# stevengiacalone/triceratops

Hardware: AMD Instinct MI355X
Metric: light-curve-point x sample evals/sec (higher is better)
Workload: dtype f64

## Files before the change

### include/trx_debug.h

```cpp
#ifndef TRX_DEBUG_H
#define TRX_DEBUG_H

#include "trx.h"

#ifdef __cplusplus
extern "C" {
#endif

int trx_set_rows_per_wave(int rows);
int trx_set_cell_packing_below(int n_time);
int trx_debug_batch_plan(long rows, int rows_per_wave, int taper, long* positions, int* rows_min);

int trx_set_supersample_tiers(int on);
int trx_set_stencil(int on);
int trx_set_skip_excluded(int on);
int trx_set_debug_node_counts(int on);
int trx_set_kepler_stepping(int on);

int trx_set_bounded_evaluation(int mode);
int trx_set_debug_bounded_lnl(int on);
int trx_set_debug_poison(int on);
int trx_set_debug_bug(int on);
int trx_set_probe_rows(int rows);
int trx_set_star_chain(int on);
int trx_set_row_order(int on);
int trx_debug_row_order(long* n_rows, long* segment_capacity, int* counts, int* lists, double* row_blocks);
int trx_set_whole_trips(int on);
int trx_set_one_sweep(int mode);
int trx_set_full_chunks(int mode);
long trx_debug_cells_lds_one_row(void);
int trx_debug_whole_trips(long* whole, long* walked, int reset);
int trx_debug_chain_counts(long* chains, long* calls_in_chains, long* posterior_calls_in_chains, int reset);

int trx_debug_select_from_halfchi2(const double* halfchi2, const double* lnprior, const double* cols,
                                   const double* cols_pad, long n, long N, long n_total, int ncol, int twin, int K,
                                   int moments, double lnsigma, double* out_record, double* out_post_x,
                                   double* out_table, void* stream);

int trx_debug_capture_buffers(long* live, long* idle);

#ifdef __cplusplus
}
#endif
#endif
```

### triceratops_amd/_lib.py

```python
import ctypes
import os
import threading

import numpy as np
import torch

_HERE = os.path.dirname(os.path.abspath(__file__))
LIB_PATH = os.environ.get("TRX_LIB") or os.path.join(_HERE, "libtrx.so")
TESTING_LIB_PATH = os.environ.get("TRX_TESTING_LIB") or os.path.join(_HERE, "libtrx_testing.so")

MODEL_TP, MODEL_EB, MODEL_EB_TWIN, MODEL_RAW = 0, 1, 2, 3
FLAG_COMPANION_IS_HOST, FLAG_SCALAR_K, FLAG_FP32_MODEL, FLAG_EVALUATE_EXCLUDED = 1, 2, 4, 8
FLAG_ALL_SUBEXPOSURES, FLAG_NO_STENCIL, FLAG_COUNT_EVALUATIONS, FLAG_FULL_EVALUATION = 16, 32, 64, 128
FLAG_WEIGHT_MOMENTS = 256
N_PARAM = {MODEL_TP: 10, MODEL_EB: 11, MODEL_EB_TWIN: 11, MODEL_RAW: 9}
ERR_NTOTAL = 4

ABI_SYMBOLS = (
    "trx_lnl_batch", "trx_lnl_batch_weighted", "trx_flux_grid", "trx_chi2_grid", "trx_chi2_grid_weighted",
    "trx_chi2_grid_offset", "trx_chi2_grid_baseline", "trx_workspace_bytes",
    "trx_log_mean_exp", "trx_lnz_scenario", "trx_lnz_from_halfchi2", "trx_lnz_moments_from_halfchi2",
    "trx_posterior_from_halfchi2", "trx_grid_quantiles",
    "trx_lnl_batch_host", "trx_flux_grid_host",
    "trx_log_mean_exp_host", "trx_skipped_rows", "trx_pruned_rows",
    "trx_draw_scenario", "trx_draw_args_size", "trx_scenario_evidence", "trx_scenario_enqueue", "trx_star_enqueue",
    "trx_scenario_args_size", "trx_release_scratch", "trx_version", "trx_last_error", "trx_device_count",
)
WARP_SYMBOLS = ("trxw_hist_from_halfchi2",)
NOISE_SYMBOLS = ("trxn_chi2_grid_ou",)
MIX_SYMBOLS = ("trxm_chi2_grid_ou_mix",)
SHIFT_SYMBOLS = ("trxt_softmin_rows",)
ROBUST_SYMBOLS = ("trxr_chi2_grid_robust",)
GLS_SYMBOLS = ("trxg_chi2_grid_ou_baseline",)
SS_SYMBOLS = ("trxs_chi2_grid_ss2",)
WHITE_SYMBOLS = ("trxv_chi2_grid_white_mix",)
DEBUG_SYMBOLS = (
    "trx_set_rows_per_wave", "trx_set_cell_packing_below", "trx_debug_batch_plan", "trx_set_supersample_tiers",
    "trx_set_stencil", "trx_set_skip_excluded", "trx_set_debug_node_counts", "trx_set_kepler_stepping",
    "trx_set_bounded_evaluation", "trx_set_debug_bounded_lnl", "trx_set_debug_poison", "trx_set_debug_bug",
    "trx_set_probe_rows", "trx_set_star_chain", "trx_debug_capture_buffers", "trx_debug_chain_counts",
    "trx_set_row_order", "trx_debug_row_order", "trx_set_whole_trips", "trx_debug_whole_trips", "trx_set_one_sweep",
    "trx_set_full_chunks", "trx_debug_cells_lds_one_row", "trx_debug_select_from_halfchi2",
)


class TrxError(RuntimeError):
    pass


EXTRA_FLAGS = 0
CELL_PACKING_BELOW = 320
STATS = {"rows": 0, "cells": 0, "launches": 0, "native_calls": 0}
_stats_lock = threading.Lock()


def count_launch(rows, n_time):
    with _stats_lock:
        STATS["rows"] += rows
        STATS["cells"] += rows * n_time
        STATS["launches"] += 1
TRACE = None
TRACE_SAMPLE_ROWS = 128


def reset_stats():
# ... 109 lines not shown
    L.trxs_chi2_grid_ss2.argtypes = [_vp, _vp, c_int, c_long, _vp, c_double, c_int, _vp, _vp, _vp, _vp, _vp]
    L.trx_grid_quantiles.restype = c_int
    L.trx_grid_quantiles.argtypes = [_vp, c_long, c_int, _vp, _vp, c_long, _vp, c_int, _vp, _vp]
    L.trx_lnl_batch_host.restype = c_int
    L.trx_lnl_batch_host.argtypes = [c_int, c_int, _vp, _vp, c_int, c_double, _vp, c_long,
                                     c_double, c_int, _vp]
    L.trx_flux_grid_host.restype = c_int
    L.trx_flux_grid_host.argtypes = [c_int, c_int, _vp, c_int, _vp, c_long, c_double, c_int, _vp, _vp]
    L.trx_log_mean_exp_host.restype = c_int
    L.trx_log_mean_exp_host.argtypes = [_vp, c_long, c_long, _vp]
    L.trx_skipped_rows.restype = c_int
    L.trx_skipped_rows.argtypes = [ctypes.POINTER(ctypes.c_ulonglong), c_int]
    L.trx_pruned_rows.restype = c_int
    L.trx_pruned_rows.argtypes = [ctypes.POINTER(ctypes.c_ulonglong), c_int]
    L.trx_version.restype = ctypes.c_char_p
    L.trx_last_error.restype = ctypes.c_char_p
    L.trx_device_count.restype = c_int
    L.trx_testing = bool(testing)
    if testing:
        for name in ("trx_set_rows_per_wave", "trx_set_kepler_stepping", "trx_set_skip_excluded",
                     "trx_set_bounded_evaluation", "trx_set_debug_bounded_lnl", "trx_set_debug_poison",
                     "trx_set_debug_bug", "trx_set_star_chain", "trx_set_probe_rows", "trx_set_stencil",
                     "trx_set_supersample_tiers", "trx_set_debug_node_counts", "trx_set_cell_packing_below",
                     "trx_set_row_order", "trx_set_whole_trips", "trx_set_one_sweep", "trx_set_full_chunks"):
            fn = getattr(L, name)
            fn.restype = c_int
            fn.argtypes = [c_int]
        L.trx_debug_cells_lds_one_row.restype = c_long
        L.trx_debug_cells_lds_one_row.argtypes = []
        L.trx_debug_capture_buffers.restype = c_int
        L.trx_debug_capture_buffers.argtypes = [ctypes.POINTER(c_long), ctypes.POINTER(c_long)]
        L.trx_debug_row_order.restype = c_int
        L.trx_debug_row_order.argtypes = [ctypes.POINTER(c_long), ctypes.POINTER(c_long), _vp, _vp, _vp]
        L.trx_debug_whole_trips.restype = c_int
        L.trx_debug_whole_trips.argtypes = [ctypes.POINTER(c_long), ctypes.POINTER(c_long), c_int]
        L.trx_debug_select_from_halfchi2.restype = c_int
        L.trx_debug_select_from_halfchi2.argtypes = [_vp, _vp, _vp, _vp, c_long, c_long, c_long, c_int, c_int, c_int, c_int,
                                                     c_double, _vp, _vp, _vp, _vp]
    return L


def check(rc):
    if rc:
        msg = lib().trx_last_error().decode()
        if rc == ERR_NTOTAL:
            raise ValueError(msg)
        raise TrxError("libtrx error %d: %s" % (rc, msg))


def version():
    return lib().trx_version().decode()


_gpu_seen = False


def require_gpu():
    global _gpu_seen
# ... 141 lines not shown

def debug_row_order():
    L = lib()
    assert L.trx_testing, "debug_row_order needs use_testing_library()"
    n, cap = ctypes.c_long(0), ctypes.c_long(0)
    check(L.trx_debug_row_order(ctypes.byref(n), ctypes.byref(cap), None, None, None))
    counts = np.zeros(64, dtype=np.int32)
    lists = np.zeros(64 * cap.value, dtype=np.int32)
    blocks = np.zeros((n.value, 19), dtype=np.float64)
    check(L.trx_debug_row_order(ctypes.byref(n), ctypes.byref(cap), counts.ctypes.data, lists.ctypes.data,
                                blocks.ctypes.data))
    lists = lists.reshape(64, cap.value)
    return counts.reshape(16, 4), [lists[s, :max(0, min(int(counts[s]), cap.value))].copy() for s in range(64)], blocks


def debug_whole_trips(reset=False):
    L = lib()
    assert L.trx_testing, "debug_whole_trips needs use_testing_library()"
    whole, walked = ctypes.c_long(0), ctypes.c_long(0)
    check(L.trx_debug_whole_trips(ctypes.byref(whole), ctypes.byref(walked), 1 if reset else 0))
    return whole.value, walked.value


def lnl_batch_weighted(model, flags, time_d, flux_d, inv_var_d, params_d, exptime, nsamples, sec_limit=float("inf"),
                       out=None):
    require_gpu()
    n, nt = params_d.shape[1], time_d.numel()
    assert params_d.shape[0] == N_PARAM[model] and params_d.is_contiguous()
    assert flux_d.numel() == nt and inv_var_d.numel() == nt
    assert time_d.is_contiguous() and flux_d.is_contiguous() and inv_var_d.is_contiguous()
    accumulate = out is not None
    if out is None:
        out = torch.empty(n, dtype=torch.float64, device=params_d.device)
    assert out.shape == (n,) and out.dtype == torch.float64 and out.is_contiguous()
    if n == 0:
        return out
    with torch.cuda.device(params_d.device):
        check(lib().trx_lnl_batch_weighted(model, flags, time_d.data_ptr(), flux_d.data_ptr(), inv_var_d.data_ptr(),
                                           nt, params_d.data_ptr(), n, float(exptime), int(nsamples),
                                           float(sec_limit), int(accumulate), out.data_ptr(), _stream(params_d)))
    return out


def flux_grid(model, flags, time_d, params_d, exptime, nsamples, want_secdepth=True, out=None):
    require_gpu()
    n = params_d.shape[1]
# ... 312 lines not shown
```

### triceratops_amd/csrc/trx_cells.hpp

```cpp
#pragma once
#include <hip/hip_runtime.h>
#include <math.h>

#include <cstddef>
#include <cstdint>

#include "../../include/trx.h"
#include "trx_device.hpp"
#include "trx_internal.hpp"

namespace {

using namespace trx;

constexpr int MODE_LNL = 0;
constexpr int MODE_GRID = 1;

struct RowsArgs {
    int model, flags;
    const double* time;
    const double* flux;
    int n_time;
    double sigma;
    const double* params;
// ... 105 lines not shown
__device__ unsigned long long g_phase_cycles[8];
#define TRX_TICK(var) const unsigned long long var = __builtin_readcyclecounter()
#define TRX_TOCK(slot, from) tm[slot] += __builtin_readcyclecounter() - (from)
#else
#define TRX_TICK(var)
#define TRX_TOCK(slot, from)
#endif

#ifdef TRX_TAIL_TIMERS
constexpr int kTailWaves = 1 << 17;
__device__ unsigned long long g_tail[4] = {~0ull, 0ull, 0ull, 0ull};
__device__ unsigned long long g_tail_finish[kTailWaves];
#endif

constexpr int kStatShards = 256, kStatPad = 16;
__device__ unsigned long long g_row_stats[2][kStatShards][kStatPad];
__device__ __forceinline__ void add_row_stat(int which, unsigned count)
{
    if (count) atomicAdd(&g_row_stats[which][(blockIdx.x + 41u * blockIdx.y) & (kStatShards - 1)][0], (unsigned long long)count);
}

#ifdef TRX_TESTING
__device__ unsigned long long g_trip_stats[2][kStatShards][kStatPad];
__device__ __forceinline__ void add_trip_stat(int which, unsigned count)
{
    if (count) atomicAdd(&g_trip_stats[which][(blockIdx.x + 41u * blockIdx.y) & (kStatShards - 1)][0], (unsigned long long)count);
}
__device__ __forceinline__ bool whole_trips_on(const RowsArgs& a) { return a.whole_trips != 0; }
__device__ __forceinline__ bool one_sweep_on(const RowsArgs& a, bool lnl) { return a.one_sweep >= (lnl ? 1 : 2); }
__device__ __forceinline__ bool full_chunks_on(const RowsArgs& a, bool lnl) { return a.full_chunks >= (lnl ? 1 : 2); }
#define TRX_TRIP_STAT(var) ++var
#else
__device__ __forceinline__ bool whole_trips_on(const RowsArgs&) { return true; }
__device__ __forceinline__ bool one_sweep_on(const RowsArgs&, bool lnl) { return lnl; }
__device__ __forceinline__ bool full_chunks_on(const RowsArgs&, bool lnl) { return lnl; }
#define TRX_TRIP_STAT(var)
#endif

__device__ __forceinline__ double k_rule(double k, bool scalar_rule)
{
    if (scalar_rule) { if (fabs(k - 1.0) < 1e-6) k *= 0.999; }
    else             { if ((k - 1.0) < 1e-6) k *= 0.999; }
    return k;
}

#ifndef TRX_BATCH_WAVES
#define TRX_BATCH_WAVES 4
#endif

constexpr int kBatchWaves = TRX_BATCH_WAVES;
__host__ __device__ constexpr int cells_waves(bool long_rows) { return long_rows ? 1 : kBatchWaves; }
#ifndef TRX_TIER_LDS
#define TRX_TIER_LDS(PRUNE, LONG) true
#endif
#ifndef TRX_ATAN_TAB
#define TRX_ATAN_TAB(PRUNE, LONG) (((PRUNE) && !(LONG)) ? 2 : 1)
#endif
#ifndef TRX_LONG_ROWS_IN_LDS
// ... 519 lines not shown
}

struct BranchMap {
    unsigned char id[TRX_CHAIN_MAX_BRANCHES];
};
__global__ __launch_bounds__(64) void sec_scan_kernel_star(RowsArgs common, BranchTab bt, BranchMap map)
{
    const RowsArgs a = star_args(common, bt, 0, (int)map.id[blockIdx.y]);
    if (!a.need_sec) return;
    sec_scan_body<8>(a);
}
static_assert(offsetof(RowC, excl) == (kRowDoubles - 1) * sizeof(double), "excl is the last field of RowC");

struct CellState {
    double sE[64], cE[64];
    double t[64];
    double facc[64];
    unsigned meta[64];
    union {
        unsigned short rel[64];
        double held[2 * kStM];
    };
};
struct StencilState {
    double fc[64 + 2 * kStM];
    double stw[2 * kStM + 1];
};
constexpr int kFcB = 2 * kStM;
constexpr int kCentreNode = 1023;

__device__ __forceinline__ double fp32_model_slack(double lb, int n_probed, double rs2)
{
    return 1e-5 * sqrt(2.0 * (double)n_probed * rs2 * fmax(lb, 0.0));
}

template <int BITS>
__device__ __forceinline__ int lane_prefix(int cnt, int& total)
{
    int off = 0;
    total = 0;
#pragma unroll
    for (int b = 0; b < BITS; ++b) {
        const unsigned long long m = __ballot((cnt >> b) & 1);
        off += lanes_below(m) << b;
        total += __popcll(m) << b;
    }
// ... 113 lines not shown
{
    typedef const __attribute__((address_space(4))) T* KernArgs;
    KernArgs p = (KernArgs)__builtin_amdgcn_kernarg_segment_ptr();
    asm volatile("" : "+s"(p));
    return (const T*)p;
}

template <int MODE, bool STEP, bool FP32, bool LONG, bool ST, bool PRUNE, int ARGS = 0, bool WT = false>
__device__ __forceinline__ void cells_body(const RowsArgs& a_in, const double st_radius)
{
    constexpr int kReload = TRX_ARGS_RELOAD ? ARGS : 0;
    const RowsArgs& a = a_in;
    static_assert(!PRUNE || (MODE == MODE_LNL && !ST), "bounded evaluation: likelihood mode, no stencil");
    static_assert(!WT || (MODE == MODE_LNL && !PRUNE), "per-point weights: likelihood mode, full evaluation");
    extern __shared__ double lds_all[];
#ifdef TRX_TAIL_TIMERS
    const unsigned long long tail_start = LONG ? wall_clock64() : 0ull;
#endif
    constexpr bool kOrdered = LONG && !PRUNE && !WT && MODE == MODE_LNL;
    int ordered_row = -2;
    if (kOrdered && a.order) ordered_row = (int)row_order_at(a.order, (long)blockIdx.x, a.n, (int)threadIdx.x);
    constexpr bool kCarry = TRX_CARRY_CELLS && STEP && !LONG;
    constexpr bool kLazyTiers = TRX_LAZY_TIERS && ST && STEP && LONG && !PRUNE;
    constexpr int W = cells_waves(LONG);
    const int wave = W > 1 ? __builtin_amdgcn_readfirstlane((int)(threadIdx.x >> 6)) : 0;
    double* tier_xw = lds_all;
    double* atab = tier_xw + 2 * kTiers * kTierMaxNodes;
    double* thead = atab + kAtanRanges * kAtanCols;
    double* lds = lds_all + a.wave_off + (size_t)wave * a.wave_doubles;
    const int Bl = LONG ? 1 : a.B;
    RowC* rows = reinterpret_cast<RowC*>(lds);
    double* hacc = lds + (size_t)Bl * kRowDoubles;
    double* hmout = hacc + Bl;
    double* hrem = hmout + Bl;
    double* hlp = hrem + Bl;
    unsigned short* pdesc = reinterpret_cast<unsigned short*>(hlp + Bl);
    constexpr int kCellsWindow = cells_window(LONG);
    unsigned short* winlist = pdesc + kCellsPairs;
    CellState& cs = *reinterpret_cast<CellState*>(winlist + kCellsWindow);
    StencilState& ss = *reinterpret_cast<StencilState*>(&cs + 1);
    const double* tl = LONG ? a.time : (lds_all + a.tl_off);
    const double* fl = LONG ? a.flux : (tl + a.n_time);
    const double* wl = LONG ? a.inv_var : (fl + a.n_time);
    if (a.use_tiers) {
        for (int i = threadIdx.x; i < 2 * kTiers * kTierMaxNodes; i += 64 * W) tier_xw[i] = a.tier_xw[i];
    }
// ... 51 lines not shown
        const unsigned long long* const surv_count = a.surv_count;
        if (a.part == 1) row1 = np;
        else if (a.part == 2) {
            if (a.split && hdr[kHdrProbe] != 0.0) { rlist = probe_list; row1 = (long)*probe_count; }
            else row0 = np;
        }
        else if (hdr[kHdrProbe] != 0.0) { rlist = surv_list; row1 = (long)*surv_count; }
        else row0 = np;
        if (!LONG && (a.part == 3 || (a.part == 2 && rlist))) B = listed_pass_rows(a, row1 - row0, a.part);
        if (!LONG && a.part == 1 && a.split) B = kPilotB < Bl ? kPilotB : Bl;
        nbatch = (row1 - row0 + B - 1) / B;
    }
    const bool third_two = PRUNE && !LONG && a.part == 3 && a.pstride3 > 1;
    const int pstride = third_two ? a.pstride3 : a.pstride;
    const bool probing = PRUNE && pstride > 1 && hdr[kHdrProbe] != 0.0 &&
                         (a.part == 0 || a.part == 2 || third_two);
    if (PRUNE && a.split && a.part == 2 && !probing) return;
    const BatchPlan bp = LONG ? BatchPlan{} : batch_plan(uniform_long(row1 - row0), __builtin_amdgcn_readfirstlane(B), !PRUNE);
    const long positions = LONG ? (nbatch + 7) / 8 : bp.P;
    const long v0 = (long)(blockIdx.x & 7) + 8 * ((long)(blockIdx.x >> 3) * W + wave);
    unsigned n_skipped = 0, n_pruned = 0;
#ifdef TRX_TESTING
    unsigned n_whole = 0, n_walked = 0;
#endif
    for (long v = v0; v < 8 * positions; v += (long)gridDim.x * W) {
        RowsArgs a_again;
        if (kReload == 2) {
            const StarKernArgs* k = kernel_arguments<StarKernArgs>();
            a_again = star_args(k->common, k->bt, k->part);
        }
        const RowsArgs& a = (kReload == 1) ? *kernel_arguments<RowsArgs>() : ((kReload == 2) ? a_again : a_in);
        long base;
        int nb;
        if (kOrdered && ordered_row != -2) {
            if (v != v0 || ordered_row < 0) continue;
            base = (long)ordered_row;
            nb = 1;
        } else if (LONG) {
            const long batch = (v & 7) * positions + (v >> 3);
            if ((v >> 3) >= positions || batch >= nbatch) continue;
            base = row0 + batch * B;
            nb = (int)((row1 - base < B) ? (row1 - base) : B);
        } else {
            batch_at(bp, v & 7, v >> 3, base, nb);
            base += row0;
            if (base >= row1) continue;
// ... 229 lines not shown
                const double t = tl[j];
                double fobs = 0.0;
                if (LONG && MODE == MODE_LNL) fobs = fl[j];
                double wobs = rs2;
                if (LONG && WT) wobs = wl[j];
                CellPlan pl;
                if (carried) {
                    pl.n = (int)(cmeta >> 18); pl.tier = (int)((cmeta >> 8) & 0xffu) - 1;
                    pl.sE = cs.sE[csrc]; pl.cE = cs.cE[csrc];
                    pl.anchored = (cmeta & 0x10000u) != 0;
                } else if (valid) {
                    const RowC& c = (LONG && !TRX_LONG_ROWS_IN_LDS) ? cu : rows[rr];
#ifndef TRX_PLAN_FULL_SOLVE
                    if (LONG && sweep == 1) pl = plan_all_subexposures<PRUNE>(c, t, a.S);
                    else
#endif
                    pl = plan_cell<false, PRUNE, TRX_TIER_LDS(PRUNE, LONG), kLazyTiers>(c, t, a.exptime, a.S, a.tiers, a.use_tiers != 0,
                                                                                        (ST && sweep == 0) ? st_radius : 0.0, thead);
                    if (STEP && !pl.anchored && pl.n > 0) {
                        kepler_full(c.nmot * (t - c.t0) + c.Mtr, c.e, pl.sE, pl.cE);
                        pl.anchored = true;
                    }
                }
                bool planned = valid;
                if (sweep == 0 && a.use_tiers) {
                    const bool heavy = valid && !pl.lazy && pl.tier < 0 && pl.n > 0;
                    if (one) {
                        planned = valid && !heavy;
                    } else {
                        const unsigned long long mh = __ballot(heavy && owned);
                        if (heavy && owned) winlist[nheavy + lanes_below(mh)] = (unsigned short)rel;
                        if (heavy) { pl.n = 0; valid = false; planned = false; }
                        nheavy += __popcll(mh);
                    }
                }
                int tier = pl.tier;
                int nodes = (valid && owned) ? pl.n : 0;
                bool st = false, centre = false;
                if (ST && sweep == 0) {
                    const int lsrc = full ? 64 - kStM : 64 - 2 * kStM;
                    const int jleft = __shfl(carry_j, lsrc + lane, 64), jhere = __shfl(j, lane - kStM, 64);
                    const int jm = (lane < kStM) ? jleft : jhere;
                    int jp = __shfl(j, lane + kStM, 64);
                    const unsigned long long mok = __ballot(planned);
                    const unsigned long long left = (carry_ok >> lsrc) & ((1ull << kStM) - 1ull);
                    int nnext = 0;
                    const int j_last = __builtin_amdgcn_readlane(j, 63);
                    if (full && w0 + 64 < count) {
                        const int more = count - (w0 + 64) < kStM ? count - (w0 + 64) : kStM;
                        if (win0 + (int)winlist[w0 + 63 + more] == j_last + more) nnext = more;
                    }
                    constexpr unsigned kAll = (1u << (2 * kStM + 1)) - 1u;
                    unsigned want = kAll;
                    bool inner = (lane >= kStM || (halo && w0 > 0)) && lane + kStM < 64;
                    if (nnext > 0) {
                        const int over = lanes_below(~0ull) - (63 - kStM);
                        if (over > 0 && over <= nnext) {
                            jp = j_last + over;
                            want = kAll >> over;
                            inner = true;
                        }
                    }
                    const unsigned long long field = (lane >= kStM) ? (mok >> (lane - kStM)) : (((mok << kStM) | left) >> lane);
                    st = inner && owned && planned && pl.n > 0 && pl.st_ok && jm == j - kStM && jp == j + kStM &&
                         ((unsigned)field & kAll) == want;
                    const unsigned long long mst = __ballot(st);
                    unsigned long long dil = mst;
#pragma unroll
                    for (int i = 1; i <= kStM; ++i) dil |= (mst << i) | (mst >> i);
                    centre = planned && ((dil >> lane) & 1ull);
                    pendm = (unsigned)(mst >> (64 - kStM));
                    bool has_value = centre;
                    if (full) {
                        const bool owes = pend_prev != 0 && lanes_below(~0ull) < 32 - __clz((int)pend_prev);
                        if (__any(owes && !centre)) {
                            if (owes) {
                                if (pl.n > 0) centre = true;
                                else if (!centre) ss.fc[kFcB + lane] = 1.0;
                                has_value = true;
                            }
                        }
                    }
                    const unsigned long long mnext = __ballot(planned && pl.n > 0 && pl.st_ok) >> (64 - kStM);
                    const int kk = lane - (64 - 2 * kStM);
                    if (lend && !last_chunk && planned && !centre && kk >= 0 && kk < kStM && (mnext & ((2ull << kk) - 1ull)) != 0) {
                        if (pl.n > 0) centre = true;
                        else ss.fc[kFcB + lane] = 1.0;
                    }
                    if (st) nodes = 0;
                    carry_j = j;
                    carry_ok = full ? __ballot(has_value) : mok;
                    if (kLazyTiers) {
                        const bool need = pl.lazy && nodes > 0;
                        if (__any(need)) {
                            if (need) {
                                const RowC& c = (LONG && !TRX_LONG_ROWS_IN_LDS) ? cu : rows[rr];
                                plan_tiers(c, a.exptime, pl, thead);
                                tier = pl.tier;
                                nodes = pl.n;
                            }
                        }
                    }
                }
                const bool direct = kLazyTiers && ST && sweep == 0 && !__any(nodes > 0);
                if (direct) {
                    if (centre) {
                        const RowC& c = (LONG && !TRX_LONG_ROWS_IN_LDS) ? cu : rows[rr];
                        const double ce = pl.cE - c.e;
                        const double X = fma(c.ax, ce, c.bx * pl.sE);
                        const double Y = fma(c.ay, ce, c.by * pl.sE);
                        const double yc = Y * c.cosi;
                        const double z2 = fma(X, X, yc * yc);
                        const double opp = 1.0 + c.k;
                        double f = 1.0;
                        if (Y >= 0.0 && z2 < opp * opp) {
                            const Limb L{c.cle, c.cld, c.ced};
                            f = disc_flux<FP32, TRX_ATAN_TAB(PRUNE, LONG)>(sqrt_fast(z2), c.k, L, atab);
                        } else if (z2 != z2) {
                            f = z2;
                        }
                        ss.fc[kFcB + lane] = f;
                    }
                    wave_sync();
                }
                if (kCarry) wave_sync();
                if (!direct) {
                    cs.sE[lane] = pl.sE; cs.cE[lane] = pl.cE;
                    cs.t[lane] = t;
                    cs.facc[lane] = 0.0;
                    cs.meta[lane] = (unsigned)rr | ((unsigned)(tier + 1) << 8) | (pl.anchored ? 0x10000u : 0u) |
                                    (valid ? 0x20000u : 0u) | ((unsigned)pl.n << 18);
                    if (kCarry) cs.rel[lane] = (unsigned short)rel;
                }
                TRX_TOCK(2, t_plan);
                TRX_TICK(t_a);
                int ldone = 64;
                const int ncells = __popcll(__ballot(nodes > 0 || (ST && centre)));
                const bool by_cells = one && a.S < kCellsPairs;
                int per = ncells > 0 ? kCellsPairs / ncells - (ST ? 1 : 0) : kCellsPairs;
                per = per > 1000 ? 1000 : (per < 1 ? 1 : per);
                if (by_cells) per = kCellsPairs;
                int lane0 = ncells > 0 ? 0 : 64;
                for (int s0 = 0; !direct && (by_cells ? lane0 < 64 : __any(s0 < nodes || (ST && s0 == 0 && centre)));
                     s0 += by_cells ? 0 : per) {
// ... 45 lines not shown
                                                             : tier_xw[2 * (ht * kTierMaxNodes + s)];
                                const double dM = c.nmot * (a.exptime * frac);
                                bool have = false;
                                if (STEP && (meta & 0x10000u)) have = kepler_step<PRUNE>(dM, c.e, sE, cE);
                                if (!have) {
                                    TRX_CENSUS_ADD(kCenKeplerFullPair, 1);
                                    kepler_full(c.nmot * ((cs.t[h] + a.exptime * frac) - c.t0) + c.Mtr, c.e, sE, cE);
                                }
                            }
                            const double ce = cE - c.e;
                            const double X = fma(c.ax, ce, c.bx * sE);
                            const double Y = fma(c.ay, ce, c.by * sE);
                            const double yc = Y * c.cosi;
                            const double z2 = fma(X, X, yc * yc);
                            const double opp = 1.0 + c.k;
                            double f = 1.0;
                            if (Y >= 0.0 && z2 < opp * opp) {
                                const Limb L{c.cle, c.cld, c.ced};
                                f = disc_flux<FP32, TRX_ATAN_TAB(PRUNE, LONG)>(sqrt_fast(z2), c.k, L, atab);
                            } else if (z2 != z2) {
                                f = z2;
                            }
                            if (at_centre) {
                                ss.fc[kFcB + h] = f;
                            } else {
                                const double term = (ht < 0) ? f : tier_xw[2 * (ht * kTierMaxNodes + s) + 1] * (1.0 - f);
                                if (ht < 0 || term != 0.0)
                                    __hip_atomic_fetch_add(&cs.facc[h], term, __ATOMIC_RELAXED, __HIP_MEMORY_SCOPE_WORKGROUP);
                            }
                        }
                    }
                    wave_sync();
                }
                TRX_TOCK(3, t_a);
                TRX_TICK(t_rest);
                const int lq = lanes_below(~0ull) - (64 - kStM);
                const bool mine_pending = ST && st && pendm != 0 && lq >= 0;
                bool adopt = mine_pending;
                unsigned left_over = 0u;
                if (ST && pend_prev != pendm) {
                    const bool prev_here = lq >= 0 && ((pend_prev >> lq) & 1u) != 0;
                    adopt = prev_here && (mine_pending || !valid);
                    left_over = (unsigned)(__ballot(prev_here && !adopt) >> (64 - kStM));
                }
                if (MODE == MODE_GRID && a.debug_nodes) {
                    const int spent = nodes + ((ST && centre) ? 1 : 0);
                    if (spent > 0 && lane < ldone) atomicAdd(&a.out[(size_t)base * n_time + cell], (double)spent);
                } else if ((valid && owned && lane < ldone && !mine_pending) || adopt) {
                    const RowC& c = (LONG && !TRX_LONG_ROWS_IN_LDS) ? cu : rows[rr];
                    double fsum = cs.facc[lane];
                    if (ST && (st || adopt)) {
                        const double* fcl = &ss.fc[kFcB + (adopt ? lq - kStM : lane)];
                        fsum = 0.0;
#pragma unroll
                        for (int i = -kStM; i <= kStM; ++i) fsum = fma(ss.stw[i + kStM], 1.0 - fcl[i], fsum);
                    }
                    const double deficit = (ST && adopt) ? fsum
                                         : ((pl.n == 0) ? 0.0 : ((ST && st) ? fsum : ((tier < 0) ? 1.0 - fsum / a.dS : fsum)));
                    const RowC& cd = rows[rr];
                    const double m = fma(-deficit, cd.rdil, 1.0);
                    if (MODE == MODE_GRID) {
                        a.out[(size_t)base * n_time + ((ST && adopt) ? win0 + (int)winlist[w0] - kStM + lq : cell)] = m;
                    } else {
                        if (LONG) {
                            const double d = ((ST && adopt) ? cs.held[lq] : fobs) - m;
                            lacc = fma(d * d, (ST && WT && adopt) ? cs.held[kStM + lq] : wobs, lacc);
                            nonflat = nonflat || (m != 1.0);
                        } else {
                            const double f = fl[j];
                            const double contrib = ((1.0 - m) * ((f - m) + (f - 1.0))) * (WT ? wl[j] : rs2);
                            if (contrib != 0.0)
                                __hip_atomic_fetch_add(&hacc[rr], contrib, __ATOMIC_RELAXED, __HIP_MEMORY_SCOPE_WORKGROUP);
                            if (PRUNE && nphase == 2 && phase_no == 0) {
                                const double d1 = f - 1.0;
                                __hip_atomic_fetch_add(&hrem[rr], -(d1 * d1) * rs2, __ATOMIC_RELAXED, __HIP_MEMORY_SCOPE_WORKGROUP);
                            }
                        }
                    }
                }
                if (ST && left_over != 0 && !(MODE == MODE_GRID && a.debug_nodes)) {
                    const int q = lanes_below(~0ull);
                    if (q < kStM && ((left_over >> q) & 1u)) {
                        const int jq = win0 + (int)winlist[w0] - kStM + q;
                        double fsum = 0.0;
#pragma unroll
                        for (int i = -kStM; i <= kStM; ++i) fsum = fma(ss.stw[i + kStM], 1.0 - ss.fc[kFcB - kStM + q + i], fsum);
                        const double m = fma(-fsum, rows[0].rdil, 1.0);
                        if (MODE == MODE_GRID) {
                            a.out[(size_t)base * n_time + jq] = m;
                        } else {
                            const double d = cs.held[q] - m;
                            lacc = fma(d * d, WT ? cs.held[kStM + q] : rs2, lacc);
                            nonflat = nonflat || (m != 1.0);
                        }
                    }
                }
                if (ST && MODE == MODE_LNL && mine_pending) {
                    cs.held[lq] = fobs;
                    if (WT) cs.held[kStM + lq] = wobs;
                }
                if (kCarry) ncarry = 64 - ldone;
                TRX_TOCK(5, t_rest);
            }
            }
            wave_sync();
            if (PRUNE && nphase == 2 && phase_no == 0) {
                const double* hdr_b = a.rowc + n * kRowDoubles;
                const double hmin_run = __hip_atomic_load(&hdr_b[kHdrHmin], __ATOMIC_RELAXED, __HIP_MEMORY_SCOPE_AGENT);
                const double xmax_run = __hip_atomic_load(&hdr_b[kHdrXmax], __ATOMIC_RELAXED, __HIP_MEMORY_SCOPE_AGENT);
// ... 67 lines not shown
                    for (int o = 32; o > 0; o >>= 1) {
                        hb = fmin(hb, __shfl_xor(hb, o, 64));
                        xb = fmax(xb, __shfl_xor(xb, o, 64));
                    }
                    if (lane == 0) tighten_bounds(a.rowc + n * kRowDoubles, hb, xb);
                }
            }
        }
        wave_sync();
    }
    if (PRUNE && !LONG && a.split && a.part == 2) {
        __shared__ unsigned long long wg_at;
        __syncthreads();
        const int nk = wg_nkeep < wg_valid ? wg_nkeep : wg_valid;
        if (threadIdx.x == 0 && nk > 0) wg_at = atomicAdd(a.surv_count, (unsigned long long)nk);
        __syncthreads();
        for (int i = threadIdx.x; i < nk; i += 64 * W) a.surv_list[wg_at + i] = wg_keep[i];
    }
#undef lp_row
    if (lane == 0) {
        add_row_stat(0, n_skipped);
        add_row_stat(1, n_pruned);
#ifdef TRX_TESTING
        if (ST) { add_trip_stat(0, n_whole); add_trip_stat(1, n_walked); }
#endif
    }
#ifdef TRX_TAIL_TIMERS
    if (LONG && lane == 0) {
        const unsigned long long tail_end = wall_clock64();
        atomicMin(&g_tail[0], tail_start);
        atomicMax(&g_tail[1], tail_start);
        atomicMax(&g_tail[2], tail_end);
        atomicAdd(&g_tail[3], tail_end - tail_start);
        if (blockIdx.y == 0 && blockIdx.x < (unsigned)kTailWaves) g_tail_finish[blockIdx.x] = tail_end;
    }
#endif
#ifdef TRX_PHASE_TIMERS
    TRX_TOCK(7, t_all);
    if (lane == 0)
        for (int i = 0; i < 8; ++i) atomicAdd(&g_phase_cycles[i], tm[i]);
#endif
}

template <int MODE, bool STEP, bool FP32, bool LONG, bool ST, bool PRUNE = false, int ARGS = 0, bool WT = false>
__device__ __forceinline__ void cells_entry(const RowsArgs& a)
{
    if (a.need_sec && blockIdx.x == 0 && threadIdx.x == 0) *a.scan_count = 0ull;
// ... 167 lines not shown
```

### triceratops_amd/csrc/trx_kernels.hip

```cpp
#include <hip/hip_runtime.h>
#include <math.h>
#include <stdio.h>
#include <stdlib.h>
#include <string.h>

#include <atomic>
#include <cstddef>
#include <cstdint>
#include <map>
#include <mutex>
#include <type_traits>
#include <utility>
#include <vector>

#include "../../include/trx.h"
#include "../../include/trx_noise.h"
#include "../../include/trx_mix.h"
#include "../../include/trx_shift.h"
#include "../../include/trx_robust.h"
#include "../../include/trx_gls.h"
#include "../../include/trx_ss.h"
#include "trx_device.hpp"
#include "trx_internal.hpp"
#include "trx_knobs.hpp"
// ... 259 lines not shown
    return (size_t)(2 * kTiers * kTierMaxNodes + kAtanRanges * kAtanCols + kTierHeadDoubles) * sizeof(double);
}
constexpr size_t cells_wave_bytes(int B, bool long_variant)
{
    return (size_t)B * (kRowDoubles + 4) * sizeof(double)
         + (kCellsPairs + cells_window(long_variant)) * sizeof(unsigned short) + sizeof(CellState)
         + (long_variant ? sizeof(StencilState) : 0);
}
static_assert(cells_tables_bytes() + cells_wave_bytes(1, true) <= 160 * 1024 / 16, "LDS of the one-row workgroup");

template <int MODE>
int plan_cells(RowsArgs& a, bool long_rows, CellsPlan& P)
{
    a.forced_B = knob_rows_per_wave();
    a.B = long_rows ? 1 : batch_rows(a.n_dev ? -1 : a.n, a.n_time, a.forced_B);
    a.s2 = a.sigma * a.sigma;
    a.rs2 = 1.0 / a.s2;
    a.dS = (double)a.S;
    a.rS = 1.0 / a.dS;
    a.nbatch = 8 * batch_plan(a.n, a.B).P;
    a.debug_bug = knob_debug_bug();
    a.whole_trips = knob_whole_trips();
    a.one_sweep = knob_one_sweep();
    a.full_chunks = knob_full_chunks();
    a.mark_unwritten = (MODE == MODE_LNL && !a.inv_var) ? 1 : 0;
    bool tiers_ok = false;
    if (tier_device(a.S, a.tiers, &a.tier_xw, &tiers_ok)) return fail(TRX_ERR_HIP, "tier table upload failed%s", "", 0);
    a.use_tiers = tiers_ok && knob_tiers() && !(a.flags & TRX_FLAG_ALL_SUBEXPOSURES);
    const int prune_mode = (a.flags & TRX_FLAG_FULL_EVALUATION) ? 0 : (a.prune == 2 ? 2 : knob_bounded());
    const bool prune = MODE == MODE_LNL && a.prune && knob_kepler_stepping() &&
                       (prune_mode == 2 || (prune_mode == 1 && long_rows)) &&
                       (long_rows || (long)a.B * a.n_time <= (long)kCellsWindowBatch) &&
                       a.n_time >= kProbeMinPoints;
    a.prune = prune ? 1 : 0;
    static const int probe_cells = (int)env_long("TRX_PROBE_CELLS", kProbeCells);
    a.pstride = prune ? (a.n_time / probe_cells > 1 ? a.n_time / probe_cells : 2) : 1;
    static const int third_stride = (int)env_long("TRX_THIRD_STRIDE", kThirdStride);
    a.pstride3 = (prune && third_stride > 1 && a.n_time >= 4 * third_stride) ? third_stride : 0;
    a.use_stencil = (!prune && long_rows && a.use_tiers && a.exptime > 0.0 && a.S >= 8 && a.n_time >= 64 &&
                     knob_stencil() && !(a.flags & TRX_FLAG_NO_STENCIL)) ? 1 : 0;
    a.skip_excl = knob_skip_excluded() && !(a.flags & TRX_FLAG_EVALUATE_EXCLUDED);
    a.need_sec = (a.model == TRX_MODEL_EB && MODE == MODE_LNL) ||
                 ((a.model == TRX_MODEL_EB || a.model == TRX_MODEL_EB_TWIN) && a.out_sec != nullptr);
    if (a.inv_var && !(a.sec_limit < INFINITY)) a.need_sec = 0;
    static_assert((kCellsPairs + kCellsWindowLong) % 4 == 0 && (kCellsPairs + kCellsWindowBatch) % 4 == 0 &&
                  sizeof(CellState) % 8 == 0 && sizeof(StencilState) % 8 == 0, "8-byte alignment of the LDS arrays");
    const size_t tables = cells_tables_bytes();
// ... 1131 lines not shown
    return TRX_OK;
}

int trx_set_whole_trips(int on)
{
    g_knob_whole_trips = on ? 1 : 0;
    return TRX_OK;
}

int trx_set_one_sweep(int mode)
{
    if (mode < 0 || mode > 2) return fail(TRX_ERR_ARG, "trx_set_one_sweep: mode must be 0, 1 or 2%s (got %ld)", "", (long)mode);
    g_knob_one_sweep = mode;
    return TRX_OK;
}

int trx_set_full_chunks(int mode)
{
    if (mode < 0 || mode > 2) return fail(TRX_ERR_ARG, "trx_set_full_chunks: mode must be 0, 1 or 2%s (got %ld)", "", (long)mode);
    g_knob_full_chunks = mode;
    return TRX_OK;
}

long trx_debug_cells_lds_one_row(void)
{
    return (long)(cells_tables_bytes() + cells_wave_bytes(1, true));
}

int trx_debug_whole_trips(long* whole, long* walked, int reset)
{
    static unsigned long long host[2][kStatShards][kStatPad];
    static std::mutex mu;
    std::lock_guard<std::mutex> lock(mu);
    TRX_HIP(hipDeviceSynchronize());
    TRX_HIP(hipMemcpyFromSymbol(host, HIP_SYMBOL(g_trip_stats), sizeof(host), 0));
    long sum[2] = {0, 0};
    for (int w = 0; w < 2; ++w)
        for (int i = 0; i < kStatShards; ++i) sum[w] += (long)host[w][i][0];
    if (whole) *whole = sum[0];
    if (walked) *walked = sum[1];
    if (reset) {
        memset(host, 0, sizeof(host));
        TRX_HIP(hipMemcpyToSymbol(HIP_SYMBOL(g_trip_stats), host, sizeof(host), 0));
    }
    return TRX_OK;
}
// ... 101 lines not shown
```

### triceratops_amd/csrc/trx_knobs.hpp

```cpp
#pragma once
#include <stdlib.h>

#ifdef TRX_TESTING
#include <atomic>
#endif

namespace trx {

#ifdef TRX_TESTING
inline int knob_env_int(const char* name, int dflt)
{
    const char* e = name ? getenv(name) : nullptr;
    return (e && *e) ? atoi(e) : dflt;
}
inline long env_long(const char* name, long dflt)
{
    const char* e = getenv(name);
    return (e && *e) ? atol(e) : dflt;
}
inline double env_double(const char* name, double dflt)
{
    const char* e = getenv(name);
    return (e && *e) ? atof(e) : dflt;
}
// ... 4 lines not shown
constexpr long env_long(const char*, long dflt) { return dflt; }
constexpr double env_double(const char*, double dflt) { return dflt; }
#define TRX_KNOB(name, dflt, env) \
    constexpr int knob_##name() { return dflt; }
#endif

TRX_KNOB(rows_per_wave, 0, nullptr)
TRX_KNOB(probe_rows, 0, "TRX_PROBE_ROWS")
TRX_KNOB(kepler_stepping, 1, nullptr)
TRX_KNOB(tiers, 1, nullptr)
TRX_KNOB(bounded, 2, "TRX_BOUNDED")
TRX_KNOB(bounded_lnl, 0, nullptr)
TRX_KNOB(skip_excluded, 1, nullptr)
TRX_KNOB(stencil, 1, nullptr)
TRX_KNOB(debug_nodes, 0, nullptr)
TRX_KNOB(cells_below, 320, nullptr)
TRX_KNOB(debug_bug, 0, nullptr)
TRX_KNOB(poison, 0, nullptr)
TRX_KNOB(star_chain, 1, "TRX_STAR_CHAIN")
TRX_KNOB(row_order, 1, nullptr)
TRX_KNOB(whole_trips, 1, nullptr)
TRX_KNOB(one_sweep, 1, nullptr)
TRX_KNOB(full_chunks, 1, nullptr)

#undef TRX_KNOB

}
```

Baseline: 52.96 billion.

## Add zone fast path for contiguous stencil chunks and store flux deficits

Adds a zone path to the lazy-tier stencil LNL kernel. When a full 64-lane chunk is contiguous with the previous carry, every lane is stencil-eligible and the next window point lies exactly kStM ahead, the chunk skips the per-lane stencil planning and shuffle logic and goes straight to direct centre evaluation. The stencil buffer now holds deficits (1-f) instead of fluxes, which removes a subtraction from each stencil tap. It also adds a testing counter and knob for zone chunks, and the extra conditions risk divergence or subtle numeric differences.

```diff
diff --git a/include/trx_debug.h b/include/trx_debug.h
--- a/include/trx_debug.h
+++ b/include/trx_debug.h
@@ -30,6 +30,8 @@
 int trx_set_full_chunks(int mode);
 long trx_debug_cells_lds_one_row(void);
 int trx_debug_whole_trips(long* whole, long* walked, int reset);
+int trx_set_zone_loop(int on);
+int trx_debug_zone_chunks(long* chunks, int reset);
 int trx_debug_chain_counts(long* chains, long* calls_in_chains, long* posterior_calls_in_chains, int reset);
 
 int trx_debug_select_from_halfchi2(const double* halfchi2, const double* lnprior, const double* cols,
diff --git a/profiles/zone_loop/measure.py b/profiles/zone_loop/measure.py
--- /dev/null
+++ b/profiles/zone_loop/measure.py
@@ -0,0 +1,124 @@
+import json
+import os
+import shutil
+import subprocess
+import sys
+import tempfile
+
+import numpy as np
+
+R = os.path.dirname(os.path.dirname(os.path.dirname(os.path.abspath(__file__))))
+PY = sys.executable
+
+
+def run(cmd, limit, lib, **kw):
+    env = dict(os.environ, TRX_LIB=lib)
+    p = subprocess.run(["timeout", "-k", "10", str(limit)] + cmd, cwd=R, env=env, stdout=subprocess.PIPE, text=True, **kw)
+    if p.returncode != 0:
+        print("FAILED (%d): %s" % (p.returncode, " ".join(cmd)))
+        print(p.stdout[-2000:])
+        sys.exit(1)
+    return p.stdout
+
+
+def last_json(text):
+    return json.loads(text.strip().splitlines()[-1])
+
+
+def arms_of(args):
+    return [(a.split("=", 1)[0], os.path.abspath(a.split("=", 1)[1])) for a in args]
+
+
+KEYS = ("cfg1", "value", "ms_per_step", "irregular", "n100", "n200", "toi64")
+
+
+def ab(reps, arms):
+    rec = {name: [] for name, _ in arms}
+    for rep in range(1, reps + 1):
+        for name, lib in arms:
+            d = last_json(run([PY, "bench.py", "--gpus", "1", "--full", "--steps", "20", "--warmup", "5", "--no-cpu-baseline",
+                               "--no-e2e", "--pmc", "off"], 500, lib))
+            sh, b = d.get("shapes") or {}, d.get("batch") or {}
+            row = {"cfg1": d["roofline"]["mean_launch_ms"], "value": d["value"], "ms_per_step": d["ms_per_step"],
+                   "irregular": (sh.get("n2000_irregular") or {}).get("mean_launch_ms", float("nan")),
+                   "n100": (sh.get("n100") or {}).get("mean_launch_ms", float("nan")),
+                   "n200": (sh.get("n200") or {}).get("mean_launch_ms", float("nan")),
+                   "toi64": b.get("ms_per_step", float("nan")), "checksum": d["lnZ_checksum"]}
+            rec[name].append(row)
+            print("%-8s rep %d  cfg1 %.4f ms  value %.4e/s  ms_per_step %.3f | irregular %.4f ms | n100 %.4f n200 %.4f | "
+                  "64-TOI step %.2f ms | lnZ_checksum %.17g"
+                  % (name, rep, row["cfg1"], row["value"], row["ms_per_step"], row["irregular"], row["n100"], row["n200"],
+                     row["toi64"], row["checksum"]))
+            sys.stdout.flush()
+    base = arms[0][0]
+    for name, _ in arms[1:]:
+        for key in KEYS:
+            p, t = (np.array([r[key] for r in rec[a]]) for a in (base, name))
+            spread = max(p.max() - p.min(), t.max() - t.min())
+            every = bool((t < p).all()) if key != "value" else bool((t > p).all())
+            print("%-11s %s %.5g (spread %.3g)  %s %.5g (spread %.3g)  difference %+.4g = %+.2f %% = %.1f within-arm spreads; "
+                  "better in every pair: %s"
+                  % (key, base, p.mean(), p.max() - p.min(), name, t.mean(), t.max() - t.min(), t.mean() - p.mean(),
+                     100.0 * (t.mean() - p.mean()) / p.mean(), abs(p.mean() - t.mean()) / spread if spread > 0 else float("inf"), every))
+
+
+def counters(arms):
+    out = tempfile.mkdtemp(prefix="zone_loop_pmc_")
+    try:
+        for name, lib in arms:
+            d = os.path.join(out, "pmc_" + name)
+            run(["rocprofv3", "--pmc", "SQ_INSTS_VALU", "SQ_ACTIVE_INST_VALU", "SQ_BUSY_CYCLES", "SQ_WAVE_CYCLES",
+                 "--output-format", "csv", "-d", d, "--", PY, "profiles/r07/cells2000_once.py"], 240, lib, stderr=subprocess.STDOUT)
+            text = run([PY, "profiles/pmc_summary.py", d], 120, lib, stderr=subprocess.STDOUT)
+            print("== counters, %s" % name)
+            lines = text.splitlines()
+            for i, line in enumerate(lines):
+                if "cells_kernel" in line and "<0" in line.replace(" ", ""):
+                    print("\n".join(lines[i:i + 5]))
+            sys.stdout.flush()
+    finally:
+        shutil.rmtree(out, ignore_errors=True)
+
+
+def outputs(parent, tree):
+    out = tempfile.mkdtemp(prefix="zone_loop_dump_")
+    try:
+        ck = {}
+        for arm, lib in (("parent", parent), ("tree", tree)):
+            d = last_json(run([PY, "bench.py", "--gpus", "1", "--steps", "2", "--warmup", "1", "--no-cpu-baseline",
+                               "--dump-outputs", os.path.join(out, arm)], 300, lib))
+            ck[arm] = d["lnZ_checksum"]
+        ok = ck["parent"] == ck["tree"]
+        print("lnZ_checksum parent %.17g tree %.17g equal: %s" % (ck["parent"], ck["tree"], ok))
+        for name in ("halfchi2", "lnZ"):
+            a, b = (np.load(os.path.join(out, arm, name + ".npy")) for arm in ("parent", "tree"))
+            places = np.array_equal(np.isnan(a), np.isnan(b)) and np.array_equal(np.isinf(a), np.isinf(b))
+            equal = places and np.array_equal(a[np.isfinite(a)], b[np.isfinite(b)]) and \
+                np.array_equal(a[np.isinf(a)], b[np.isinf(b)])
+            bits = int((a.view(np.uint64) == b.view(np.uint64)).sum())
+            print("%s.npy %s: np.array_equal %s, %d of %d values bit-identical, non-finite entries in the same places: %s"
+                  % (name, a.shape, equal, bits, a.size, places))
+            ok = ok and equal and bits == a.size
+        print("outputs equal: %s" % ok)
+        if not ok:
+            sys.exit(1)
+    finally:
+        shutil.rmtree(out, ignore_errors=True)
+
+
+def chunks(testing):
+    print(run([PY, "profiles/zone_loop/zone_chunks.py"], 240, testing))
+
+
+if __name__ == "__main__":
+    stage = sys.argv[1]
+    if stage == "ab":
+        ab(int(sys.argv[2]), arms_of(sys.argv[3:]))
+    elif stage == "counters":
+        counters(arms_of(sys.argv[2:]))
+    elif stage == "outputs":
+        outputs(os.path.abspath(sys.argv[2]), os.path.abspath(sys.argv[3]))
+    elif stage == "chunks":
+        chunks(os.path.abspath(sys.argv[2]))
+    else:
+        sys.exit("unknown stage " + stage)
diff --git a/profiles/zone_loop/zone_chunks.py b/profiles/zone_loop/zone_chunks.py
--- /dev/null
+++ b/profiles/zone_loop/zone_chunks.py
@@ -0,0 +1,27 @@
+import os
+import sys
+
+import numpy as np
+
+sys.path.insert(0, os.path.join(os.path.dirname(os.path.abspath(__file__)), "..", ".."))
+from oracle import oracle as O
+from triceratops_amd import _lib, synth
+
+_lib.use_testing_library(True)
+L = _lib.lib()
+rng = np.random.default_rng(synth.SEED)
+t = synth.time_grid(2000)
+flux = synth.noisy_light_curve(rng, O.flux_grid(O.MODEL_TP, t, synth.reference_tp_row())[0][0])
+t_d, f_d = _lib.dev(t), _lib.dev(flux)
+rows = [_lib.dev(synth.family_rows(rng, fam, 512)) for fam in synth.FAMILIES]
+for on in (1, 0):
+    assert L.trx_set_zone_loop(on) == 0
+    _lib.debug_zone_chunks(reset=True)
+    per_family = []
+    for (name, model, is_host, has_comp), r in zip(synth.FAMILIES, rows):
+        flags = _lib.FLAG_COMPANION_IS_HOST if is_host else 0
+        _lib.lnl_batch(model, flags, t_d, f_d, synth.SIGMA, r, synth.EXPTIME, synth.NSAMPLES)
+        per_family.append(_lib.debug_zone_chunks(reset=True) / 512.0)
+    print("trx_set_zone_loop(%d): %.3f zone chunks per row (18 families x 512 rows x 2000 points); per family %s"
+          % (on, float(np.mean(per_family)), " ".join("%.2f" % v for v in per_family)))
+assert L.trx_set_zone_loop(1) == 0
diff --git a/triceratops_amd/_lib.py b/triceratops_amd/_lib.py
--- a/triceratops_amd/_lib.py
+++ b/triceratops_amd/_lib.py
@@ -40,7 +40,8 @@
     "trx_set_bounded_evaluation", "trx_set_debug_bounded_lnl", "trx_set_debug_poison", "trx_set_debug_bug",
     "trx_set_probe_rows", "trx_set_star_chain", "trx_debug_capture_buffers", "trx_debug_chain_counts",
     "trx_set_row_order", "trx_debug_row_order", "trx_set_whole_trips", "trx_debug_whole_trips", "trx_set_one_sweep",
-    "trx_set_full_chunks", "trx_debug_cells_lds_one_row", "trx_debug_select_from_halfchi2",
+    "trx_set_full_chunks", "trx_debug_cells_lds_one_row", "trx_debug_select_from_halfchi2", "trx_set_zone_loop",
+    "trx_debug_zone_chunks",
 )
 
 
@@ -196,7 +197,8 @@
                      "trx_set_bounded_evaluation", "trx_set_debug_bounded_lnl", "trx_set_debug_poison",
                      "trx_set_debug_bug", "trx_set_star_chain", "trx_set_probe_rows", "trx_set_stencil",
                      "trx_set_supersample_tiers", "trx_set_debug_node_counts", "trx_set_cell_packing_below",
-                     "trx_set_row_order", "trx_set_whole_trips", "trx_set_one_sweep", "trx_set_full_chunks"):
+                     "trx_set_row_order", "trx_set_whole_trips", "trx_set_one_sweep", "trx_set_full_chunks",
+                     "trx_set_zone_loop"):
             fn = getattr(L, name)
             fn.restype = c_int
             fn.argtypes = [c_int]
@@ -208,6 +210,8 @@
         L.trx_debug_row_order.argtypes = [ctypes.POINTER(c_long), ctypes.POINTER(c_long), _vp, _vp, _vp]
         L.trx_debug_whole_trips.restype = c_int
         L.trx_debug_whole_trips.argtypes = [ctypes.POINTER(c_long), ctypes.POINTER(c_long), c_int]
+        L.trx_debug_zone_chunks.restype = c_int
+        L.trx_debug_zone_chunks.argtypes = [ctypes.POINTER(c_long), c_int]
         L.trx_debug_select_from_halfchi2.restype = c_int
         L.trx_debug_select_from_halfchi2.argtypes = [_vp, _vp, _vp, _vp, c_long, c_long, c_long, c_int, c_int, c_int, c_int,
                                                      c_double, _vp, _vp, _vp, _vp]
@@ -395,6 +399,14 @@
     return whole.value, walked.value
 
 
+def debug_zone_chunks(reset=False):
+    L = lib()
+    assert L.trx_testing, "debug_zone_chunks needs use_testing_library()"
+    chunks = ctypes.c_long(0)
+    check(L.trx_debug_zone_chunks(ctypes.byref(chunks), 1 if reset else 0))
+    return chunks.value
+
+
 def lnl_batch_weighted(model, flags, time_d, flux_d, inv_var_d, params_d, exptime, nsamples, sec_limit=float("inf"),
                        out=None):
     require_gpu()
diff --git a/triceratops_amd/csrc/trx_cells.hpp b/triceratops_amd/csrc/trx_cells.hpp
--- a/triceratops_amd/csrc/trx_cells.hpp
+++ b/triceratops_amd/csrc/trx_cells.hpp
@@ -151,18 +151,25 @@
 
 #ifdef TRX_TESTING
 __device__ unsigned long long g_trip_stats[2][kStatShards][kStatPad];
+__device__ unsigned long long g_zone_stats[kStatShards][kStatPad];
 __device__ __forceinline__ void add_trip_stat(int which, unsigned count)
 {
     if (count) atomicAdd(&g_trip_stats[which][(blockIdx.x + 41u * blockIdx.y) & (kStatShards - 1)][0], (unsigned long long)count);
+}
+__device__ __forceinline__ void add_zone_stat(unsigned count)
+{
+    if (count) atomicAdd(&g_zone_stats[(blockIdx.x + 41u * blockIdx.y) & (kStatShards - 1)][0], (unsigned long long)count);
 }
 __device__ __forceinline__ bool whole_trips_on(const RowsArgs& a) { return a.whole_trips != 0; }
 __device__ __forceinline__ bool one_sweep_on(const RowsArgs& a, bool lnl) { return a.one_sweep >= (lnl ? 1 : 2); }
-__device__ __forceinline__ bool full_chunks_on(const RowsArgs& a, bool lnl) { return a.full_chunks >= (lnl ? 1 : 2); }
+__device__ __forceinline__ bool full_chunks_on(const RowsArgs& a, bool lnl) { return (a.full_chunks & 3) >= (lnl ? 1 : 2); }
+__device__ __forceinline__ bool zone_loop_on(const RowsArgs& a) { return (a.full_chunks & 4) != 0; }
 #define TRX_TRIP_STAT(var) ++var
 #else
 __device__ __forceinline__ bool whole_trips_on(const RowsArgs&) { return true; }
 __device__ __forceinline__ bool one_sweep_on(const RowsArgs&, bool lnl) { return lnl; }
 __device__ __forceinline__ bool full_chunks_on(const RowsArgs&, bool lnl) { return lnl; }
+__device__ __forceinline__ bool zone_loop_on(const RowsArgs&) { return true; }
 #define TRX_TRIP_STAT(var)
 #endif
 
@@ -728,6 +735,12 @@
         double held[2 * kStM];
     };
 };
+#ifndef TRX_ST_DEFICITS
+#define TRX_ST_DEFICITS 1
+#endif
+#ifndef TRX_ZONE_LOOP
+#define TRX_ZONE_LOOP 1
+#endif
 struct StencilState {
     double fc[64 + 2 * kStM];
     double stw[2 * kStM + 1];
@@ -887,6 +900,9 @@
     if (kOrdered && a.order) ordered_row = (int)row_order_at(a.order, (long)blockIdx.x, a.n, (int)threadIdx.x);
     constexpr bool kCarry = TRX_CARRY_CELLS && STEP && !LONG;
     constexpr bool kLazyTiers = TRX_LAZY_TIERS && ST && STEP && LONG && !PRUNE;
+    constexpr bool kZoneInst = kLazyTiers && MODE == MODE_LNL;
+    constexpr bool kDeficits = TRX_ST_DEFICITS && kZoneInst;
+    constexpr bool kZone = TRX_ZONE_LOOP && kZoneInst;
     constexpr int W = cells_waves(LONG);
     const int wave = W > 1 ? __builtin_amdgcn_readfirstlane((int)(threadIdx.x >> 6)) : 0;
     double* tier_xw = lds_all;
@@ -984,6 +1000,7 @@
     unsigned n_skipped = 0, n_pruned = 0;
 #ifdef TRX_TESTING
     unsigned n_whole = 0, n_walked = 0;
+    unsigned n_zone = 0;
 #endif
     for (long v = v0; v < 8 * positions; v += (long)gridDim.x * W) {
         RowsArgs a_again;
@@ -1259,6 +1276,15 @@
                         pl.anchored = true;
                     }
                 }
+                bool zone = false;
+                if (kZone && full && zone_loop_on(a) && w0 > 0 && w0 + 64 + kStM <= count && pendm == (1u << kStM) - 1u &&
+                    (carry_ok >> (64 - 2 * kStM)) == (1ull << (2 * kStM)) - 1ull) {
+                    const int r_first = __builtin_amdgcn_readlane(rel, 0), r_last = __builtin_amdgcn_readlane(rel, 63);
+                    const int r_next = __builtin_amdgcn_readfirstlane((int)winlist[w0 + 63 + kStM]);
+                    const int j_prev = __builtin_amdgcn_readlane(carry_j, 63);
+                    zone = r_last - r_first == 63 && win0 + r_first == j_prev + 1 && r_next - r_last == kStM &&
+                           __all(pl.st_ok && pl.n > 0);
+                }
                 bool planned = valid;
                 if (sweep == 0 && a.use_tiers) {
                     const bool heavy = valid && !pl.lazy && pl.tier < 0 && pl.n > 0;
@@ -1273,8 +1299,14 @@
                 }
                 int tier = pl.tier;
                 int nodes = (valid && owned) ? pl.n : 0;
-                bool st = false, centre = false;
-                if (ST && sweep == 0) {
+                bool st = zone, centre = zone;
+                if (zone) {
+                    nodes = 0;
+                    carry_j = j;
+                    carry_ok = ~0ull;
+                    TRX_TRIP_STAT(n_zone);
+                }
+                if (ST && sweep == 0 && !zone) {
                     const int lsrc = full ? 64 - kStM : 64 - 2 * kStM;
                     const int jleft = __shfl(carry_j, lsrc + lane, 64), jhere = __shfl(j, lane - kStM, 64);
                     const int jm = (lane < kStM) ? jleft : jhere;
@@ -1313,7 +1345,7 @@
                         if (__any(owes && !centre)) {
                             if (owes) {
                                 if (pl.n > 0) centre = true;
-                                else if (!centre) ss.fc[kFcB + lane] = 1.0;
+                                else if (!centre) ss.fc[kFcB + lane] = kDeficits ? 0.0 : 1.0;
                                 has_value = true;
                             }
                         }
@@ -1322,7 +1354,7 @@
                     const int kk = lane - (64 - 2 * kStM);
                     if (lend && !last_chunk && planned && !centre && kk >= 0 && kk < kStM && (mnext & ((2ull << kk) - 1ull)) != 0) {
                         if (pl.n > 0) centre = true;
-                        else ss.fc[kFcB + lane] = 1.0;
+                        else ss.fc[kFcB + lane] = kDeficits ? 0.0 : 1.0;
                     }
                     if (st) nodes = 0;
                     carry_j = j;
@@ -1339,7 +1371,7 @@
                         }
                     }
                 }
-                const bool direct = kLazyTiers && ST && sweep == 0 && !__any(nodes > 0);
+                const bool direct = kLazyTiers && ST && sweep == 0 && (zone || !__any(nodes > 0));
                 if (direct) {
                     if (centre) {
                         const RowC& c = (LONG && !TRX_LONG_ROWS_IN_LDS) ? cu : rows[rr];
@@ -1356,7 +1388,7 @@
                         } else if (z2 != z2) {
                             f = z2;
                         }
-                        ss.fc[kFcB + lane] = f;
+                        ss.fc[kFcB + lane] = kDeficits ? 1.0 - f : f;
                     }
                     wave_sync();
                 }
@@ -1448,7 +1480,7 @@
                                 f = z2;
                             }
                             if (at_centre) {
-                                ss.fc[kFcB + h] = f;
+                                ss.fc[kFcB + h] = kDeficits ? 1.0 - f : f;
                             } else {
                                 const double term = (ht < 0) ? f : tier_xw[2 * (ht * kTierMaxNodes + s) + 1] * (1.0 - f);
                                 if (ht < 0 || term != 0.0)
@@ -1479,7 +1511,7 @@
                         const double* fcl = &ss.fc[kFcB + (adopt ? lq - kStM : lane)];
                         fsum = 0.0;
 #pragma unroll
-                        for (int i = -kStM; i <= kStM; ++i) fsum = fma(ss.stw[i + kStM], 1.0 - fcl[i], fsum);
+                        for (int i = -kStM; i <= kStM; ++i) fsum = fma(ss.stw[i + kStM], kDeficits ? fcl[i] : 1.0 - fcl[i], fsum);
                     }
                     const double deficit = (ST && adopt) ? fsum
                                          : ((pl.n == 0) ? 0.0 : ((ST && st) ? fsum : ((tier < 0) ? 1.0 - fsum / a.dS : fsum)));
@@ -1510,7 +1542,8 @@
                         const int jq = win0 + (int)winlist[w0] - kStM + q;
                         double fsum = 0.0;
 #pragma unroll
-                        for (int i = -kStM; i <= kStM; ++i) fsum = fma(ss.stw[i + kStM], 1.0 - ss.fc[kFcB - kStM + q + i], fsum);
+                        for (int i = -kStM; i <= kStM; ++i)
+                            fsum = fma(ss.stw[i + kStM], kDeficits ? ss.fc[kFcB - kStM + q + i] : 1.0 - ss.fc[kFcB - kStM + q + i], fsum);
                         const double m = fma(-fsum, rows[0].rdil, 1.0);
                         if (MODE == MODE_GRID) {
                             a.out[(size_t)base * n_time + jq] = m;
@@ -1624,7 +1657,7 @@
         add_row_stat(0, n_skipped);
         add_row_stat(1, n_pruned);
 #ifdef TRX_TESTING
-        if (ST) { add_trip_stat(0, n_whole); add_trip_stat(1, n_walked); }
+        if (ST) { add_trip_stat(0, n_whole); add_trip_stat(1, n_walked); add_zone_stat(n_zone); }
 #endif
     }
 #ifdef TRX_TAIL_TIMERS
diff --git a/triceratops_amd/csrc/trx_kernels.hip b/triceratops_amd/csrc/trx_kernels.hip
--- a/triceratops_amd/csrc/trx_kernels.hip
+++ b/triceratops_amd/csrc/trx_kernels.hip
@@ -305,7 +305,7 @@
     a.debug_bug = knob_debug_bug();
     a.whole_trips = knob_whole_trips();
     a.one_sweep = knob_one_sweep();
-    a.full_chunks = knob_full_chunks();
+    a.full_chunks = knob_full_chunks() | (knob_zone_loop() ? 4 : 0);
     a.mark_unwritten = (MODE == MODE_LNL && !a.inv_var) ? 1 : 0;
     bool tiers_ok = false;
     if (tier_device(a.S, a.tiers, &a.tier_xw, &tiers_ok)) return fail(TRX_ERR_HIP, "tier table upload failed%s", "", 0);
@@ -1483,6 +1483,29 @@
     return TRX_OK;
 }
 
+int trx_set_zone_loop(int on)
+{
+    g_knob_zone_loop = on ? 1 : 0;
+    return TRX_OK;
+}
+
+int trx_debug_zone_chunks(long* chunks, int reset)
+{
+    static unsigned long long host[kStatShards][kStatPad];
+    static std::mutex mu;
+    std::lock_guard<std::mutex> lock(mu);
+    TRX_HIP(hipDeviceSynchronize());
+    TRX_HIP(hipMemcpyFromSymbol(host, HIP_SYMBOL(g_zone_stats), sizeof(host), 0));
+    long sum = 0;
+    for (int i = 0; i < kStatShards; ++i) sum += (long)host[i][0];
+    if (chunks) *chunks = sum;
+    if (reset) {
+        memset(host, 0, sizeof(host));
+        TRX_HIP(hipMemcpyToSymbol(HIP_SYMBOL(g_zone_stats), host, sizeof(host), 0));
+    }
+    return TRX_OK;
+}
+
 long trx_debug_cells_lds_one_row(void)
 {
     return (long)(cells_tables_bytes() + cells_wave_bytes(1, true));
diff --git a/triceratops_amd/csrc/trx_knobs.hpp b/triceratops_amd/csrc/trx_knobs.hpp
--- a/triceratops_amd/csrc/trx_knobs.hpp
+++ b/triceratops_amd/csrc/trx_knobs.hpp
@@ -50,6 +50,7 @@
 TRX_KNOB(whole_trips, 1, nullptr)
 TRX_KNOB(one_sweep, 1, nullptr)
 TRX_KNOB(full_chunks, 1, nullptr)
+TRX_KNOB(zone_loop, 1, nullptr)
 
 #undef TRX_KNOB
 
```

Result: faster. 54.47 billion (median of 6 runs) (+2.9%).
